# aws-neuron/neuronx-distributed

Measured on AMD Instinct MI355X. Metric: tokens/sec (whole node) Llama-2-7B training, TP=num_gpus, seq=4096, higher is better.
Workload: dtype bf16; 1 GPU; model=llama2-7b, global_batch=32, seq_len=4096, parallelism=tp1, zero1=True

## Files before the change

### neuronx_distributed_amd/ops/csrc/flash_attn.hip

```cpp

#include "common.h"
#include "mfma.h"

#define FA_D 128
#define FA_QW 32
#define FA_WAVES 8
#define FA_QBLK (FA_QW * FA_WAVES)
#define FA_KV 64
#define LOG2E 1.4426950408889634f
#define NEG_INF (-1e30f)

#define K_TILE_B (FA_KV * FA_D * 2)
#define VT_PITCH 72
#define VT_TILE_B (FA_D * VT_PITCH * 2)

extern "C" __global__ void __launch_bounds__(512, 2)
flash_fwd_kernel(const short* __restrict__ qp, const short* __restrict__ kp,
                 const short* __restrict__ vp, short* __restrict__ op,
                 float* __restrict__ lsep, int B, int Hq, int Hkv, int S,
                 float scale, int causal, int window,
                 long q_bs, long q_hs, long q_ss,
                 long k_bs, long k_hs, long k_ss,
                 long v_bs, long v_hs, long v_ss,
                 long o_bs, long o_hs, long o_ss) {
  extern __shared__ __attribute__((aligned(16))) char smem[];
  auto kbuf = [&](int i) { return smem + (size_t)i * K_TILE_B; };
  auto vbuf = [&](int i) {
    return smem + 3 * K_TILE_B + (size_t)i * VT_TILE_B;
  };

  const int lane = threadIdx.x & 63;
  const int wid = __builtin_amdgcn_readfirstlane(threadIdx.x >> 6);
  const int col = lane & 31;
  const int hi = lane >> 5;

  const int qblk = (int)(gridDim.y - 1 - blockIdx.y);
  const int h = blockIdx.x;
  const int b = blockIdx.z;
  const int hkv = h / (Hq / Hkv);

  const long q_base = (long)b * q_bs + (long)h * q_hs;
  const long kv_base_k = (long)b * k_bs + (long)hkv * k_hs;
  const long kv_base_v = (long)b * v_bs + (long)hkv * v_hs;

  const int q0 = qblk * FA_QBLK;
  const int qw0 = q0 + wid * FA_QW;
  const int my_q = qw0 + col;
  const int q_row_ld = my_q < S ? my_q : S - 1;

  frag_u qf[8];
#pragma unroll
  for (int c = 0; c < 8; ++c) {
    const short* src = qp + q_base + (long)q_row_ld * q_ss + c * 16 + hi * 8;
    qf[c].u4 = *(const uint4v*)src;
  }

  f32x16 ot[4] = {};
  float m_run = NEG_INF;
  float l_run = 0.f;

  const int kv_end = causal ? min(S, q0 + FA_QBLK) : S;
  const int ntiles = (kv_end + FA_KV - 1) / FA_KV;
  const int my_kv_end = causal ? min(S, qw0 + FA_QW) : S;
  const int my_kv_begin = window > 0 ? max(0, qw0 - window + 1) : 0;
  const int t_begin = window > 0 ? max(0, q0 - window + 1) / FA_KV : 0;

  const float s2 = scale * LOG2E;

  const int tid = threadIdx.x;
  const int st_rp = tid >> 4;
  const int st_c16 = tid & 15;
  const int st_r0 = 2 * st_rp, st_r1 = 2 * st_rp + 1;

  uint4v kreg[2], vreg[2];
  auto issue_loads = [&](int t) {
    int kv0 = t * FA_KV;
    int rr0 = kv0 + st_r0 < S ? kv0 + st_r0 : S - 1;
    int rr1 = kv0 + st_r1 < S ? kv0 + st_r1 : S - 1;
    kreg[0] = *(const uint4v*)(kp + kv_base_k + (long)rr0 * k_ss + st_c16 * 8);
    kreg[1] = *(const uint4v*)(kp + kv_base_k + (long)rr1 * k_ss + st_c16 * 8);
    vreg[0] = *(const uint4v*)(vp + kv_base_v + (long)rr0 * v_ss + st_c16 * 8);
    vreg[1] = *(const uint4v*)(vp + kv_base_v + (long)rr1 * v_ss + st_c16 * 8);
  };

  auto write_tile = [&](int buf) {
    *(uint4v*)(kbuf(buf) + swz16(st_r0, st_c16 * 16)
               + st_r0 * (FA_D * 2)) = kreg[0];
    *(uint4v*)(kbuf(buf) + swz16(st_r1, st_c16 * 16)
               + st_r1 * (FA_D * 2)) = kreg[1];
    union { uint4v u; short s[8]; } a, b;
    a.u = vreg[0];
    b.u = vreg[1];
#pragma unroll
    for (int j = 0; j < 8; ++j) {
      int d = st_c16 * 8 + j;
      uint pair = ((uint)(unsigned short)a.s[j]) |
                  (((uint)(unsigned short)b.s[j]) << 16);
      *(uint*)(vbuf(buf) + d * (VT_PITCH * 2) + st_r0 * 2) = pair;
    }
  };

  issue_loads(t_begin);
  write_tile(t_begin % 3);
  __syncthreads();

  for (int t = t_begin; t < ntiles; ++t) {
    const int kv0 = t * FA_KV;
    const int cur = t % 3;
    if (t + 1 < ntiles) issue_loads(t + 1);

    const bool wave_active = kv0 < my_kv_end &&
        (window <= 0 || kv0 + FA_KV > my_kv_begin);
    if (wave_active) {
      f32x16 acc[2] = {};
      frag_u kfr[2][8];
#pragma unroll
      for (int kb = 0; kb < 2; ++kb) {
        int row = col + 32 * kb;
#pragma unroll
        for (int c = 0; c < 8; ++c)
          kfr[kb][c].u4 = *(const uint4v*)(kbuf(cur) + row * (FA_D * 2)
                                           + swz16(row, (c * 16 + hi * 8) * 2));
      }
      __builtin_amdgcn_s_setprio(1);
#pragma unroll
      for (int kb = 0; kb < 2; ++kb)
#pragma unroll
        for (int c = 0; c < 8; ++c)
          acc[kb] = mfma_bf16(kfr[kb][c].bf, qf[c].bf, acc[kb]);
      __builtin_amdgcn_s_setprio(0);

      float sc[2][16];
      const bool need_mask =
          (causal && kv0 + FA_KV > qw0) || (kv0 + FA_KV > S) ||
          (window > 0 && kv0 < qw0 + FA_QW - 1 - window + 1 + FA_KV);
#pragma unroll
      for (int kb = 0; kb < 2; ++kb)
#pragma unroll
        for (int r = 0; r < 16; ++r) {
          float v = acc[kb][r] * s2;
          if (need_mask) {
            int kg = kv0 + 32 * kb + acc_row(r, hi);
            if ((causal && kg > my_q) || kg >= S ||
                (window > 0 && kg <= my_q - window)) v = NEG_INF;
          }
          sc[kb][r] = v;
        }

      float mt = NEG_INF;
#pragma unroll
      for (int kb = 0; kb < 2; ++kb)
#pragma unroll
        for (int r = 0; r < 16; ++r) mt = fmaxf(mt, sc[kb][r]);
      mt = fmaxf(mt, __shfl_xor(mt, 32, 64));

      float m_new = fmaxf(m_run, mt);
      float m_eff = fmaxf(m_new, -1e28f);
      float alpha = __builtin_amdgcn_exp2f(m_run - m_eff);
      m_run = m_new;

      float psum = 0.f;
#pragma unroll
      for (int kb = 0; kb < 2; ++kb)
#pragma unroll
        for (int r = 0; r < 16; ++r) {
          float p = __builtin_amdgcn_exp2f(sc[kb][r] - m_eff);
          sc[kb][r] = p;
          psum += p;
        }
      psum += __shfl_xor(psum, 32, 64);
      l_run = l_run * alpha + psum;

#pragma unroll
      for (int nb = 0; nb < 4; ++nb) ot[nb] *= alpha;

      frag_u pf[4];
#pragma unroll
      for (int kb = 0; kb < 2; ++kb)
#pragma unroll
        for (int cc = 0; cc < 2; ++cc) {
          uint b0 = pack_bf16x2(sc[kb][8 * cc + 0], sc[kb][8 * cc + 1]);
          uint b1 = pack_bf16x2(sc[kb][8 * cc + 2], sc[kb][8 * cc + 3]);
          uint b2 = pack_bf16x2(sc[kb][8 * cc + 4], sc[kb][8 * cc + 5]);
          uint b3 = pack_bf16x2(sc[kb][8 * cc + 6], sc[kb][8 * cc + 7]);
          {
            auto r01 = __builtin_amdgcn_permlane32_swap(b0, b2, false, false);
            b0 = r01[0]; b2 = r01[1];
          }
          {
            auto r23 = __builtin_amdgcn_permlane32_swap(b1, b3, false, false);
            b1 = r23[0]; b3 = r23[1];
          }
          frag_u& f = pf[2 * kb + cc];
          f.u[0] = b0; f.u[1] = b1; f.u[2] = b2; f.u[3] = b3;
        }

#pragma unroll
      for (int np = 0; np < 2; ++np) {
        frag_u vfr[2][4];
#pragma unroll
        for (int ni = 0; ni < 2; ++ni) {
          int d = 32 * (2 * np + ni) + col;
#pragma unroll
          for (int c16 = 0; c16 < 4; ++c16)
            vfr[ni][c16].u4 = *(const uint4v*)(vbuf(cur) + d * (VT_PITCH * 2)
                                               + (c16 * 16 + hi * 8) * 2);
        }
        __builtin_amdgcn_s_setprio(1);
#pragma unroll
        for (int ni = 0; ni < 2; ++ni)
#pragma unroll
          for (int c16 = 0; c16 < 4; ++c16)
            ot[2 * np + ni] =
                mfma_bf16(vfr[ni][c16].bf, pf[c16].bf, ot[2 * np + ni]);
        __builtin_amdgcn_s_setprio(0);
      }
    }

    if (t + 1 < ntiles) write_tile((t + 1) % 3);
    __syncthreads();
  }

  if (my_q >= S) return;
  float inv_l = l_run > 0.f ? 1.f / l_run : 0.f;
  long o_row = (long)b * o_bs + (long)h * o_hs + (long)my_q * o_ss;
#pragma unroll
  for (int nb = 0; nb < 4; ++nb) {
#pragma unroll
    for (int rg = 0; rg < 4; ++rg) {
      int d = 32 * nb + 8 * rg + 4 * hi;
      uint w0 = pack_bf16x2(ot[nb][4 * rg + 0] * inv_l,
                            ot[nb][4 * rg + 1] * inv_l);
      uint w1 = pack_bf16x2(ot[nb][4 * rg + 2] * inv_l,
                            ot[nb][4 * rg + 3] * inv_l);
      uint2 st = {w0, w1};
      *(uint2*)(op + o_row + d) = st;
    }
  }
  if (hi == 0 && lsep) {
    lsep[(long)(b * Hq + h) * S + my_q] =
        m_run * 0.6931471805599453f + __logf(l_run);
  }
}

extern "C" void flash_attn_fwd(const void* q, const void* k, const void* v,
                               void* out, void* lse, int B, int Hq, int Hkv,
                               int S, float scale, int causal,
                               hipStream_t stream) {
  dim3 grid(Hq, (S + FA_QBLK - 1) / FA_QBLK, B);
  size_t lds = 3 * (K_TILE_B + VT_TILE_B);
  flash_fwd_kernel<<<grid, 512, lds, stream>>>(
      (const short*)q, (const short*)k, (const short*)v, (short*)out,
      (float*)lse, B, Hq, Hkv, S, scale, causal, 0,
      (long)Hq * S * FA_D, (long)S * FA_D, FA_D,
      (long)Hkv * S * FA_D, (long)S * FA_D, FA_D,
      (long)Hkv * S * FA_D, (long)S * FA_D, FA_D,
      (long)Hq * S * FA_D, (long)S * FA_D, FA_D);
}

extern "C" void flash_attn_fwd_strided(
    const void* q, const void* k, const void* v, void* out, void* lse,
    int B, int Hq, int Hkv, int S, float scale, int causal, int window,
    const long* st, hipStream_t stream) {
  dim3 grid(Hq, (S + FA_QBLK - 1) / FA_QBLK, B);
  size_t lds = 3 * (K_TILE_B + VT_TILE_B);
  flash_fwd_kernel<<<grid, 512, lds, stream>>>(
      (const short*)q, (const short*)k, (const short*)v, (short*)out,
      (float*)lse, B, Hq, Hkv, S, scale, causal, window,
      st[0], st[1], st[2], st[3], st[4], st[5], st[6], st[7], st[8],
      st[9], st[10], st[11]);
}

extern "C" void flash_attn_fwd_window(const void* q, const void* k,
                                      const void* v, void* out, void* lse,
                                      int B, int Hq, int Hkv, int S,
                                      float scale, int window,
                                      hipStream_t stream) {
  dim3 grid(Hq, (S + FA_QBLK - 1) / FA_QBLK, B);
  size_t lds = 3 * (K_TILE_B + VT_TILE_B);
  flash_fwd_kernel<<<grid, 512, lds, stream>>>(
      (const short*)q, (const short*)k, (const short*)v, (short*)out,
      (float*)lse, B, Hq, Hkv, S, scale, 1, window,
      (long)Hq * S * FA_D, (long)S * FA_D, FA_D,
      (long)Hkv * S * FA_D, (long)S * FA_D, FA_D,
      (long)Hkv * S * FA_D, (long)S * FA_D, FA_D,
      (long)Hq * S * FA_D, (long)S * FA_D, FA_D);
}
```

### neuronx_distributed_amd/ops/csrc/mfma.h

```cpp
#pragma once

#include "common.h"

typedef __bf16 bf16x8 __attribute__((ext_vector_type(8)));
typedef float f32x16 __attribute__((ext_vector_type(16)));
typedef unsigned int uint4v __attribute__((ext_vector_type(4)));

__device__ __forceinline__ f32x16 mfma_bf16(bf16x8 a, bf16x8 b, f32x16 c) {
  return __builtin_amdgcn_mfma_f32_32x32x16_bf16(a, b, c, 0, 0, 0);
}

union frag_u {
  bf16x8 bf;
  uint4v u4;
  uint u[4];
};

__device__ __forceinline__ int acc_row(int r, int hi) {
  return (r & 3) + 8 * (r >> 2) + 4 * hi;
}

__device__ __forceinline__ uint pack_bf16x2(float lo, float hi) {
  union { __bf16 b[2]; uint u; } r;
  r.b[0] = (__bf16)lo;
  r.b[1] = (__bf16)hi;
  return r.u;
}

__device__ __forceinline__ int swz(int row, int byte_in_row) {
  return byte_in_row ^ ((row & 7) << 4);
}

__device__ __forceinline__ int swz16(int row, int byte_in_row) {
  return byte_in_row ^ ((row & 15) << 4);
}

#define IMG_ROW_B 256

__device__ __forceinline__ int img_off(int row, int ch) {
  return IMG_ROW_B * row + 16 * (ch ^ (((row & 3) << 2) | ((row >> 2) & 3)));
}


__device__ __forceinline__ int img_row_base(int row, int hi) {
  return img_off(row, hi);
}
__device__ __forceinline__ uint4v img_row_read(const char* img, int base,
                                               int c) {
  return *(const uint4v*)(img + (base ^ (32 * c)));
}

typedef short s4v_t __attribute__((ext_vector_type(4)));
__device__ __forceinline__ int img_tr_base(int lane) {
  const int i = lane & 15;
  const int q = i >> 2, p = i & 3;
  return img_off(8 * (lane >> 5) + q, 2 * ((lane >> 4) & 1) + (p >> 1)) +
         8 * (p & 1);
}
__device__ __forceinline__ uint4v img_tr_read(const char* img, int base,
                                              int k0, int n0) {
  typedef __attribute__((address_space(3))) s4v_t lds_s4v;
  union { s4v_t s[2]; uint4v u4; } r;
  r.s[0] = __builtin_amdgcn_ds_read_tr16_b64_v4i16(
      (lds_s4v*)(img + (base ^ (2 * n0)) + IMG_ROW_B * k0));
  r.s[1] = __builtin_amdgcn_ds_read_tr16_b64_v4i16(
      (lds_s4v*)(img + (base ^ (2 * n0) ^ 16) + IMG_ROW_B * (k0 + 4)));
  return r.u4;
}
```

Before: 23820 tokens/s.

## Store V untransposed in LDS and read via ds_read_tr; double-buffer tiles

Replaces the per-element transposed V staging in LDS with a swizzled row image and uses ds_read_tr16_b64 transpose reads to build the V fragments, so V goes in with four 16-byte stores instead of many 4-byte stores. K/V buffers drop from triple to double buffering, and V fragments are loaded ahead of the softmax so the loads overlap with it. Masking is made branch-free, and the output is staged through LDS for coalesced 16-byte global stores. The changes raise register pressure from holding all V fragments at once and depend on the layout of the transposing LDS read being correct.

```diff
diff --git a/neuronx_distributed_amd/ops/csrc/flash_attn.hip b/neuronx_distributed_amd/ops/csrc/flash_attn.hip
--- a/neuronx_distributed_amd/ops/csrc/flash_attn.hip
+++ b/neuronx_distributed_amd/ops/csrc/flash_attn.hip
@@ -10,9 +10,10 @@
 #define LOG2E 1.4426950408889634f
 #define NEG_INF (-1e30f)
 
-#define K_TILE_B (FA_KV * FA_D * 2)
-#define VT_PITCH 72
-#define VT_TILE_B (FA_D * VT_PITCH * 2)
+#define FA_TILE_B (FA_KV * IMG_ROW_B)
+#define FA_BUF_B (2 * FA_TILE_B)
+#define FA_LDS_V FA_TILE_B
+#define FA_LDS_TOTAL (2 * FA_BUF_B)
 
 extern "C" __global__ void __launch_bounds__(512, 2)
 flash_fwd_kernel(const short* __restrict__ qp, const short* __restrict__ kp,
@@ -24,10 +25,6 @@
                  long v_bs, long v_hs, long v_ss,
                  long o_bs, long o_hs, long o_ss) {
   extern __shared__ __attribute__((aligned(16))) char smem[];
-  auto kbuf = [&](int i) { return smem + (size_t)i * K_TILE_B; };
-  auto vbuf = [&](int i) {
-    return smem + 3 * K_TILE_B + (size_t)i * VT_TILE_B;
-  };
 
   const int lane = threadIdx.x & 63;
   const int wid = __builtin_amdgcn_readfirstlane(threadIdx.x >> 6);
@@ -84,44 +81,41 @@
   };
 
   auto write_tile = [&](int buf) {
-    *(uint4v*)(kbuf(buf) + swz16(st_r0, st_c16 * 16)
-               + st_r0 * (FA_D * 2)) = kreg[0];
-    *(uint4v*)(kbuf(buf) + swz16(st_r1, st_c16 * 16)
-               + st_r1 * (FA_D * 2)) = kreg[1];
-    union { uint4v u; short s[8]; } a, b;
-    a.u = vreg[0];
-    b.u = vreg[1];
-#pragma unroll
-    for (int j = 0; j < 8; ++j) {
-      int d = st_c16 * 8 + j;
-      uint pair = ((uint)(unsigned short)a.s[j]) |
-                  (((uint)(unsigned short)b.s[j]) << 16);
-      *(uint*)(vbuf(buf) + d * (VT_PITCH * 2) + st_r0 * 2) = pair;
-    }
+    char* kimg = smem + buf * FA_BUF_B;
+    char* vimg = kimg + FA_LDS_V;
+    *(uint4v*)(kimg + img_off(st_r0, st_c16)) = kreg[0];
+    *(uint4v*)(kimg + img_off(st_r1, st_c16)) = kreg[1];
+    *(uint4v*)(vimg + img_off(st_r0, st_c16)) = vreg[0];
+    *(uint4v*)(vimg + img_off(st_r1, st_c16)) = vreg[1];
   };
 
+  const int row_base = img_row_base(col, hi);
+  const int tr_base = img_tr_base(lane) + FA_LDS_V;
+
   issue_loads(t_begin);
-  write_tile(t_begin % 3);
+  write_tile(0);
   __syncthreads();
-
-  for (int t = t_begin; t < ntiles; ++t) {
+#pragma unroll
+  for (int c = 0; c < 8; ++c) asm volatile("" : "+v"(qf[c].u4));
+
+  int cur = 0;
+  for (int t = t_begin; t < ntiles; ++t, cur ^= 1) {
     const int kv0 = t * FA_KV;
-    const int cur = t % 3;
     if (t + 1 < ntiles) issue_loads(t + 1);
 
     const bool wave_active = kv0 < my_kv_end &&
         (window <= 0 || kv0 + FA_KV > my_kv_begin);
     if (wave_active) {
+      const int rowb = row_base + cur * FA_BUF_B;
+      const int trb = tr_base + cur * FA_BUF_B;
       f32x16 acc[2] = {};
       frag_u kfr[2][8];
 #pragma unroll
-      for (int kb = 0; kb < 2; ++kb) {
-        int row = col + 32 * kb;
+      for (int kb = 0; kb < 2; ++kb)
 #pragma unroll
         for (int c = 0; c < 8; ++c)
-          kfr[kb][c].u4 = *(const uint4v*)(kbuf(cur) + row * (FA_D * 2)
-                                           + swz16(row, (c * 16 + hi * 8) * 2));
-      }
+          kfr[kb][c].u4 =
+              img_row_read(smem, rowb + kb * (32 * IMG_ROW_B), c);
       __builtin_amdgcn_s_setprio(1);
 #pragma unroll
       for (int kb = 0; kb < 2; ++kb)
@@ -130,22 +124,32 @@
           acc[kb] = mfma_bf16(kfr[kb][c].bf, qf[c].bf, acc[kb]);
       __builtin_amdgcn_s_setprio(0);
 
+      frag_u vfr[4][4];
+#pragma unroll
+      for (int c16 = 0; c16 < 4; ++c16)
+#pragma unroll
+        for (int nb = 0; nb < 4; ++nb)
+          vfr[c16][nb].u4 = img_tr_read(smem, trb, 16 * c16, 32 * nb);
+
       float sc[2][16];
+#pragma unroll
+      for (int kb = 0; kb < 2; ++kb)
+#pragma unroll
+        for (int r = 0; r < 16; ++r) sc[kb][r] = acc[kb][r] * s2;
       const bool need_mask =
           (causal && kv0 + FA_KV > qw0) || (kv0 + FA_KV > S) ||
           (window > 0 && kv0 < qw0 + FA_QW - 1 - window + 1 + FA_KV);
-#pragma unroll
-      for (int kb = 0; kb < 2; ++kb)
-#pragma unroll
-        for (int r = 0; r < 16; ++r) {
-          float v = acc[kb][r] * s2;
-          if (need_mask) {
+      if (need_mask) {
+#pragma unroll
+        for (int kb = 0; kb < 2; ++kb)
+#pragma unroll
+          for (int r = 0; r < 16; ++r) {
             int kg = kv0 + 32 * kb + acc_row(r, hi);
-            if ((causal && kg > my_q) || kg >= S ||
-                (window > 0 && kg <= my_q - window)) v = NEG_INF;
+            bool masked = ((causal != 0) & (kg > my_q)) | (kg >= S) |
+                ((window > 0) & (kg <= my_q - window));
+            sc[kb][r] = masked ? NEG_INF : sc[kb][r];
           }
-          sc[kb][r] = v;
-        }
+      }
 
       float mt = NEG_INF;
 #pragma unroll
@@ -158,85 +162,79 @@
       float m_eff = fmaxf(m_new, -1e28f);
       float alpha = __builtin_amdgcn_exp2f(m_run - m_eff);
       m_run = m_new;
+#pragma unroll
+      for (int nb = 0; nb < 4; ++nb) ot[nb] *= alpha;
 
       float psum = 0.f;
-#pragma unroll
-      for (int kb = 0; kb < 2; ++kb)
-#pragma unroll
-        for (int r = 0; r < 16; ++r) {
-          float p = __builtin_amdgcn_exp2f(sc[kb][r] - m_eff);
-          sc[kb][r] = p;
+      frag_u pf[4];
+      auto p_chunk = [&](int s) {
+        const int kb = s >> 1, r0 = 8 * (s & 1);
+#pragma unroll
+        for (int j = 0; j < 8; ++j) {
+          float p = __builtin_amdgcn_exp2f(sc[kb][r0 + j] - m_eff);
+          sc[kb][r0 + j] = p;
           psum += p;
         }
+        uint b0 = pack_bf16x2(sc[kb][r0 + 0], sc[kb][r0 + 1]);
+        uint b1 = pack_bf16x2(sc[kb][r0 + 2], sc[kb][r0 + 3]);
+        uint b2 = pack_bf16x2(sc[kb][r0 + 4], sc[kb][r0 + 5]);
+        uint b3 = pack_bf16x2(sc[kb][r0 + 6], sc[kb][r0 + 7]);
+        {
+          auto r01 = __builtin_amdgcn_permlane32_swap(b0, b2, false, false);
+          b0 = r01[0]; b2 = r01[1];
+        }
+        {
+          auto r23 = __builtin_amdgcn_permlane32_swap(b1, b3, false, false);
+          b1 = r23[0]; b3 = r23[1];
+        }
+        pf[s].u[0] = b0; pf[s].u[1] = b1; pf[s].u[2] = b2; pf[s].u[3] = b3;
+      };
+#pragma unroll
+      for (int s = 0; s < 4; ++s) p_chunk(s);
+      __builtin_amdgcn_s_setprio(1);
+#pragma unroll
+      for (int nb = 0; nb < 4; ++nb)
+#pragma unroll
+        for (int c16 = 0; c16 < 4; ++c16)
+          ot[nb] = mfma_bf16(vfr[c16][nb].bf, pf[c16].bf, ot[nb]);
+      __builtin_amdgcn_s_setprio(0);
       psum += __shfl_xor(psum, 32, 64);
       l_run = l_run * alpha + psum;
-
-#pragma unroll
-      for (int nb = 0; nb < 4; ++nb) ot[nb] *= alpha;
-
-      frag_u pf[4];
-#pragma unroll
-      for (int kb = 0; kb < 2; ++kb)
-#pragma unroll
-        for (int cc = 0; cc < 2; ++cc) {
-          uint b0 = pack_bf16x2(sc[kb][8 * cc + 0], sc[kb][8 * cc + 1]);
-          uint b1 = pack_bf16x2(sc[kb][8 * cc + 2], sc[kb][8 * cc + 3]);
-          uint b2 = pack_bf16x2(sc[kb][8 * cc + 4], sc[kb][8 * cc + 5]);
-          uint b3 = pack_bf16x2(sc[kb][8 * cc + 6], sc[kb][8 * cc + 7]);
-          {
-            auto r01 = __builtin_amdgcn_permlane32_swap(b0, b2, false, false);
-            b0 = r01[0]; b2 = r01[1];
-          }
-          {
-            auto r23 = __builtin_amdgcn_permlane32_swap(b1, b3, false, false);
-            b1 = r23[0]; b3 = r23[1];
-          }
-          frag_u& f = pf[2 * kb + cc];
-          f.u[0] = b0; f.u[1] = b1; f.u[2] = b2; f.u[3] = b3;
-        }
-
-#pragma unroll
-      for (int np = 0; np < 2; ++np) {
-        frag_u vfr[2][4];
-#pragma unroll
-        for (int ni = 0; ni < 2; ++ni) {
-          int d = 32 * (2 * np + ni) + col;
-#pragma unroll
-          for (int c16 = 0; c16 < 4; ++c16)
-            vfr[ni][c16].u4 = *(const uint4v*)(vbuf(cur) + d * (VT_PITCH * 2)
-                                               + (c16 * 16 + hi * 8) * 2);
-        }
-        __builtin_amdgcn_s_setprio(1);
-#pragma unroll
-        for (int ni = 0; ni < 2; ++ni)
-#pragma unroll
-          for (int c16 = 0; c16 < 4; ++c16)
-            ot[2 * np + ni] =
-                mfma_bf16(vfr[ni][c16].bf, pf[c16].bf, ot[2 * np + ni]);
-        __builtin_amdgcn_s_setprio(0);
+    }
+
+    if (t + 1 < ntiles) write_tile(cur ^ 1);
+    __syncthreads();
+  }
+
+  float inv_l = l_run > 0.f ? 1.f / l_run : 0.f;
+  long o_base = (long)b * o_bs + (long)h * o_hs;
+  if (qw0 < S) {
+    char* otile = smem + wid * (FA_QW * IMG_ROW_B);
+#pragma unroll
+    for (int nb = 0; nb < 4; ++nb) {
+#pragma unroll
+      for (int rg = 0; rg < 4; ++rg) {
+        uint w0 = pack_bf16x2(ot[nb][4 * rg + 0] * inv_l,
+                              ot[nb][4 * rg + 1] * inv_l);
+        uint w1 = pack_bf16x2(ot[nb][4 * rg + 2] * inv_l,
+                              ot[nb][4 * rg + 3] * inv_l);
+        uint2 st = {w0, w1};
+        *(uint2*)(otile + img_off(col, 4 * nb + rg) + 8 * hi) = st;
       }
     }
-
-    if (t + 1 < ntiles) write_tile((t + 1) % 3);
-    __syncthreads();
-  }
-
+    __builtin_amdgcn_s_waitcnt(0);
+#pragma unroll
+    for (int i = 0; i < 8; ++i) {
+      int p = lane + i * 64;
+      int row = p >> 4, c16 = p & 15;
+      int qg = qw0 + row;
+      if (qg < S) {
+        uint4v vv = *(const uint4v*)(otile + img_off(row, c16));
+        *(uint4v*)(op + o_base + (long)qg * o_ss + c16 * 8) = vv;
+      }
+    }
+  }
   if (my_q >= S) return;
-  float inv_l = l_run > 0.f ? 1.f / l_run : 0.f;
-  long o_row = (long)b * o_bs + (long)h * o_hs + (long)my_q * o_ss;
-#pragma unroll
-  for (int nb = 0; nb < 4; ++nb) {
-#pragma unroll
-    for (int rg = 0; rg < 4; ++rg) {
-      int d = 32 * nb + 8 * rg + 4 * hi;
-      uint w0 = pack_bf16x2(ot[nb][4 * rg + 0] * inv_l,
-                            ot[nb][4 * rg + 1] * inv_l);
-      uint w1 = pack_bf16x2(ot[nb][4 * rg + 2] * inv_l,
-                            ot[nb][4 * rg + 3] * inv_l);
-      uint2 st = {w0, w1};
-      *(uint2*)(op + o_row + d) = st;
-    }
-  }
   if (hi == 0 && lsep) {
     lsep[(long)(b * Hq + h) * S + my_q] =
         m_run * 0.6931471805599453f + __logf(l_run);
@@ -248,7 +246,7 @@
                                int S, float scale, int causal,
                                hipStream_t stream) {
   dim3 grid(Hq, (S + FA_QBLK - 1) / FA_QBLK, B);
-  size_t lds = 3 * (K_TILE_B + VT_TILE_B);
+  size_t lds = FA_LDS_TOTAL;
   flash_fwd_kernel<<<grid, 512, lds, stream>>>(
       (const short*)q, (const short*)k, (const short*)v, (short*)out,
       (float*)lse, B, Hq, Hkv, S, scale, causal, 0,
@@ -263,7 +261,7 @@
     int B, int Hq, int Hkv, int S, float scale, int causal, int window,
     const long* st, hipStream_t stream) {
   dim3 grid(Hq, (S + FA_QBLK - 1) / FA_QBLK, B);
-  size_t lds = 3 * (K_TILE_B + VT_TILE_B);
+  size_t lds = FA_LDS_TOTAL;
   flash_fwd_kernel<<<grid, 512, lds, stream>>>(
       (const short*)q, (const short*)k, (const short*)v, (short*)out,
       (float*)lse, B, Hq, Hkv, S, scale, causal, window,
@@ -277,7 +275,7 @@
                                       float scale, int window,
                                       hipStream_t stream) {
   dim3 grid(Hq, (S + FA_QBLK - 1) / FA_QBLK, B);
-  size_t lds = 3 * (K_TILE_B + VT_TILE_B);
+  size_t lds = FA_LDS_TOTAL;
   flash_fwd_kernel<<<grid, 512, lds, stream>>>(
       (const short*)q, (const short*)k, (const short*)v, (short*)out,
       (float*)lse, B, Hq, Hkv, S, scale, 1, window,
diff --git a/neuronx_distributed_amd/ops/csrc/mfma.h b/neuronx_distributed_amd/ops/csrc/mfma.h
--- a/neuronx_distributed_amd/ops/csrc/mfma.h
+++ b/neuronx_distributed_amd/ops/csrc/mfma.h
@@ -29,10 +29,6 @@
 
 __device__ __forceinline__ int swz(int row, int byte_in_row) {
   return byte_in_row ^ ((row & 7) << 4);
-}
-
-__device__ __forceinline__ int swz16(int row, int byte_in_row) {
-  return byte_in_row ^ ((row & 15) << 4);
 }
 
 #define IMG_ROW_B 256
```

Measured after the change: 24140 tokens/s, median of 6. 1.3% higher.
